# PaddlePaddle/MetaGym

Hardware: NVIDIA H100
Metric: env-steps/sec (quadrotor 6-DoF, 65k envs) (higher is better)
Workload: dtype f32

## Files before the change

metagym_b200/csrc/quad.cu:

```cuda
#include <math.h>
#include <stdlib.h>
#include <string.h>
#include <new>
#include <vector>

#include "mgb_common.cuh"
#include "quad_lanes.cuh"

namespace {

constexpr int kThreads = 64;
constexpr int kMaxObs = 19;

struct QuadConst {
    float h;
    float k1phi;
    float k1;
    float inv_phi;
    float hjm;
    float hk;
    float mm;
    float ct0, ct1, ct2;
    float vmin, vmax;
    float A[4], B[4];
// ... 691 lines not shown
    TargetRows<T> tr;
    int ct_now[N];
#pragma unroll
    for (int h = 0; h < N; ++h) {
        s.ct[h] += 1;
        ct_now[h] = s.ct[h];
    }
    const bool vel = c.task == MGB_TASK_VELOCITY_CONTROL;
    if (EARLY && vel) {
#pragma unroll
        for (int h = 0; h < N; ++h) prefetch_targets(c, a, task[h], ct_now[h], h, tr);
    }
    const T z_old = vadd(s.p[2], c.z_off);
    const T x_old = s.p[0], y_old = s.p[1];
    int fail[N];
    if (N == 1 && c.rk4_steps > 0) {
        QState s1;
        get_lane_state(s, 0, s1);
        float adj1[9], id1, pw1;
        fail[0] = integrate_rk4<SIMPLE>(c, s1, make_float4(lane(V[0], 0), lane(V[1], 0), lane(V[2], 0), lane(V[3], 0)),
                                        adj1, id1, pw1);
        set_lane_state(s, 0, s1);
#pragma unroll
        for (int k = 0; k < 9; ++k) set_lane(adj[k], 0, adj1[k]);
        set_lane(id, 0, id1);
        set_lane(power, 0, pw1);
    } else {
        const bool failed = integrate<SIMPLE, T>(c, s, V, adj, id, power, fail);
        if (N > 1 && failed) {
#pragma unroll 1
            for (int h = 0; h < N; ++h) {
                QState s1;
                load_state(a, e + h, s1);
                float adj1[9], id1, pw1;
                adjugate(s1.R, adj1, id1);
                const float V1[4] = {lane(V[0], h), lane(V[1], h), lane(V[2], h), lane(V[3], h)};
                int f1[1];
                integrate<SIMPLE, float>(c, s1, V1, adj1, id1, pw1, f1);
                s1.ct[0] = s.ct[h];
                s1.ep[0] = s.ep[h];
                set_lane_state(s, h, s1);
#pragma unroll
                for (int k = 0; k < 9; ++k) set_lane(adj[k], h, adj1[k]);
                set_lane(id, h, id1);
                set_lane(power, h, pw1);
                fail[h] = f1[0];
            }
        }
    }
    if (!EARLY && vel) {
#pragma unroll
        for (int h = 0; h < N; ++h) prefetch_targets(c, a, task[h], ct_now[h], h, tr);
    }
    const bool state_first = N == 1 && STATE_FIRST && vel;
    if (state_first) {
        QState s1;
        get_lane_state(s, 0, s1);
        if (s1.ct[0] == c.nt || fail[0]) s1.ct[0] = 0;
        store_state(a, e, s1);
    }
    T o[kMaxObs], reward;
    int done[N], trunc[N];
    bool wf[N];
    finish_step(c, a, e, s, adj, id, z_old, x_old, y_old, power, fail, tr, o, reward, done, wf, trunc);
    bool stored = false;
    if constexpr (N == 2) {
        if (nact == 2) {
            store_state2(a, e, s);
            *reinterpret_cast<float2 *>(a.rew + e) = reward.v;
            *reinterpret_cast<uchar2 *>(a.done + e) = make_uchar2((uint8_t)done[0], (uint8_t)done[1]);
            if (a.fail) *reinterpret_cast<int2 *>(a.fail + e) = make_int2(fail[0], fail[1]);
            if (a.truncated) *reinterpret_cast<uchar2 *>(a.truncated + e) = make_uchar2((uint8_t)trunc[0], (uint8_t)trunc[1]);
            stored = true;
        }
    }
    if (!stored) {
#pragma unroll
        for (int h = 0; h < N; ++h) {
            if (h < nact) {
                QState s1;
                get_lane_state(s, h, s1);
                if (!state_first || wf[h]) store_state(a, e + h, s1);
                a.rew[e + h] = lane(reward, h);
                a.done[e + h] = (uint8_t)done[h];
                if (a.fail) a.fail[e + h] = fail[h];
                if (a.truncated) a.truncated[e + h] = (uint8_t)trunc[h];
            }
        }
    }
#pragma unroll
    for (int h = 0; h < N; ++h) {
        if (h < nact) {
            float *tr_h = trow + h * D;
            if (wf[h]) {
                if (a.final_obs) {
                    float *fr_h = frow + h * D;
#pragma unroll
                    for (int k = 0; k < 16; ++k) fr_h[k] = lane(o[k], h);
                    if (D == 19) { fr_h[16] = lane(o[16], h); fr_h[17] = lane(o[17], h); fr_h[18] = lane(o[18], h); }
                    final_mask |= 1 << h;
                }
                observe_reset(c, a, task[h], s, h, o);
            }
#pragma unroll
            for (int k = 0; k < 16; ++k) tr_h[k] = lane(o[k], h);
            if (D == 19) { tr_h[16] = lane(o[16], h); tr_h[17] = lane(o[17], h); tr_h[18] = lane(o[18], h); }
        }
    }
}

__device__ __forceinline__ void publish_final(const QuadArgs &a, const float *ftile, int64_t e, int local_row, int lanes,
                                              int final_mask, int D)
{
    if (!a.final_obs) return;
    if (__syncthreads_or(final_mask)) {
        for (int h = 0; h < lanes; ++h) {
            if (final_mask & (1 << h)) {
                float *dst = a.final_obs + (e + h) * D;
                const float *frow = ftile + (local_row + h) * D;
                for (int k = 0; k < D; ++k) dst[k] = frow[k];
            }
        }
    }
}

template <bool SIMPLE>
__global__ void __launch_bounds__(kThreads) quad_step_kernel(const __grid_constant__ QuadConst c,
                                                             const __grid_constant__ QuadArgs a)
{
    __shared__ __align__(128) float tile[kThreads * kMaxObs];
    __shared__ __align__(128) float ftile[kThreads * kMaxObs];
    const int64_t e0 = (int64_t)blockIdx.x * kThreads;
    const int64_t e = e0 + threadIdx.x;
    const int rows = (int)((a.n - e0) < kThreads ? (a.n - e0) : kThreads);
    const int D = c.obs_dim;
    const bool active = e < a.n;
    int final_mask = 0;

    asm volatile("griddepcontrol.launch_dependents;");
    const int task[1] = {active ? env_task(c, a, e) : 0};
    asm volatile("griddepcontrol.wait;" ::: "memory");

    if (active) {
        QState s;
        load_state(a, e, s);
        const float4 act = __ldg(reinterpret_cast<const float4 *>(a.act) + e);
        const float V[4] = {act.x, act.y, act.z, act.w};
        step_body<SIMPLE, false, true, float>(c, a, e, 1, s, V, task, tile + threadIdx.x * D, ftile + threadIdx.x * D,
                                              final_mask);
    }
    publish_tile(a.obs, tile, e0, rows, D);
    publish_final(a, ftile, e, threadIdx.x, 1, final_mask, D);
    if (threadIdx.x == 0) mgb_bulk_wait_read<0>();
}

template <bool SIMPLE>
__global__ void __launch_bounds__(512, 1) quad_step_wide_kernel(const __grid_constant__ QuadConst c,
                                                                const __grid_constant__ QuadArgs a)
{
    extern __shared__ __align__(128) float wide_smem[];
    const int per = a.per_cta;
    float *tile = wide_smem, *ftile = wide_smem + (size_t)per * kMaxObs;
    const int64_t e0 = (int64_t)blockIdx.x * per;
    const int64_t e = e0 + threadIdx.x;
    int rows = (int)((a.n - e0) < per ? (a.n - e0) : per);
    if (rows < 0) rows = 0;
    const int D = c.obs_dim;
    const bool active = (int)threadIdx.x < rows;
    int final_mask = 0;
    asm volatile("griddepcontrol.launch_dependents;");
    const int task[1] = {active ? env_task(c, a, e) : 0};
    asm volatile("griddepcontrol.wait;" ::: "memory");
    if (active) {
        QState s;
        load_state(a, e, s);
        const float4 act = __ldg(reinterpret_cast<const float4 *>(a.act) + e);
        const float V[4] = {act.x, act.y, act.z, act.w};
        step_body<SIMPLE, false, false, float>(c, a, e, 1, s, V, task, tile + threadIdx.x * D, ftile + threadIdx.x * D,
                                               final_mask);
    }
    if (rows > 0) publish_tile(a.obs, tile, e0, rows, D);
    else __syncthreads();
    publish_final(a, ftile, e, threadIdx.x, 1, final_mask, D);
    if (threadIdx.x == 0) mgb_bulk_wait_read<0>();
}

template <bool SIMPLE>
__global__ void __launch_bounds__(256, 1) quad_step2_kernel(const __grid_constant__ QuadConst c,
                                                            const __grid_constant__ QuadArgs a)
{
    extern __shared__ __align__(128) float pair_smem[];
    const int per = a.per_cta;
    float *tile = pair_smem, *ftile = pair_smem + (size_t)per * kMaxObs;
    const int64_t e0 = (int64_t)blockIdx.x * per;
    int rows = (int)((a.n - e0) < per ? (a.n - e0) : per);
    if (rows < 0) rows = 0;
    const int le = 2 * (int)threadIdx.x;
    const int64_t e = e0 + le;
    const int D = c.obs_dim;
    const int nact = rows - le >= 2 ? 2 : (rows - le > 0 ? 1 : 0);
    int final_mask = 0;
    asm volatile("griddepcontrol.launch_dependents;");
    asm volatile("griddepcontrol.wait;" ::: "memory");
    if (nact > 0) {
        VState<f2> s;
        load_state2(a, e, s);
        const float4 a0 = __ldg(reinterpret_cast<const float4 *>(a.act) + e);
        const float4 a1 = nact == 2 ? __ldg(reinterpret_cast<const float4 *>(a.act) + e + 1) : make_float4(0.f, 0.f, 0.f, 0.f);
        const f2 V[4] = {pack2(a0.x, a1.x), pack2(a0.y, a1.y), pack2(a0.z, a1.z), pack2(a0.w, a1.w)};
        const int task[2] = {env_task(c, a, e), env_task(c, a, nact == 2 ? e + 1 : e)};
        step_body<SIMPLE, true, false, f2>(c, a, e, nact, s, V, task, tile + le * D, ftile + le * D, final_mask);
    }
    if (rows > 0) publish_tile(a.obs, tile, e0, rows, D);
    else __syncthreads();
    publish_final(a, ftile, e, le, 2, final_mask, D);
    if (threadIdx.x == 0) mgb_bulk_wait_read<0>();
}

constexpr int kStreamThreads = 128;

template <bool SIMPLE>
__global__ void __launch_bounds__(kStreamThreads, 4) quad_stream_kernel(const __grid_constant__ QuadConst c,
                                                                        const __grid_constant__ QuadArgs a)
{
    __shared__ __align__(128) float4 stage[2][7][kStreamThreads];
    __shared__ __align__(128) float tile[kStreamThreads * kMaxObs];
    __shared__ __align__(128) float ftile[kStreamThreads * kMaxObs];
    __shared__ __align__(8) uint64_t full[2];
    const int D = c.obs_dim;
    const int64_t n_tiles = (a.n + kStreamThreads - 1) / kStreamThreads;
    const int tid = threadIdx.x;

    asm volatile("griddepcontrol.launch_dependents;");
    asm volatile("griddepcontrol.wait;" ::: "memory");
    if (tid == 0) {
        mgb_mbar_init(&full[0], 1);
        mgb_mbar_init(&full[1], 1);
        mgb_fence_mbar_init();
    }
    __syncthreads();

    auto fetch = [&](int64_t t, int st) {
        const int64_t e0 = t * kStreamThreads;
        const uint32_t rows = (uint32_t)((a.n - e0) < kStreamThreads ? (a.n - e0) : kStreamThreads);
        static_assert(kStreamThreads == kTileEnvs, "one CTA iteration = one state tile");
        mgb_mbar_expect_tx(&full[st], 6u * kTileEnvs * 16u + rows * 16u);
        mgb_bulk_load(stage[st][0], a.planes + t * (6 * kTileEnvs), 6u * kTileEnvs * 16u, &full[st]);
        mgb_bulk_load(stage[st][6], reinterpret_cast<const float4 *>(a.act) + e0, rows * 16u, &full[st]);
    };

    int64_t t = blockIdx.x;
    if (tid == 0 && t < n_tiles) fetch(t, 0);
    uint32_t phase[2] = {0u, 0u};
    int st = 0;
    for (; t < n_tiles; t += gridDim.x, st ^= 1) {
        const int64_t t_next = t + gridDim.x;
        if (tid == 0 && t_next < n_tiles) fetch(t_next, st ^ 1);
        mgb_mbar_wait(&full[st], phase[st]);
        phase[st] ^= 1u;
        const int64_t e0 = t * kStreamThreads, e = e0 + tid;
        const int rows = (int)((a.n - e0) < kStreamThreads ? (a.n - e0) : kStreamThreads);
        int final_mask = 0;
        if (tid == 0) mgb_bulk_wait_read<0>();
        __syncthreads();
        if (tid < rows) {
            QState s;
            float4 q[kPlanes];
#pragma unroll
            for (int k = 0; k < kPlanes; ++k) q[k] = stage[st][k][tid];
            unpack_state(q, s);
            const float4 act = stage[st][6][tid];
            const float V[4] = {act.x, act.y, act.z, act.w};
            const int task[1] = {env_task(c, a, e)};
            step_body<SIMPLE, true, false, float>(c, a, e, 1, s, V, task, tile + tid * D, ftile + tid * D, final_mask);
        }
        publish_tile(a.obs, tile, e0, rows, D);
        publish_final(a, ftile, e, tid, 1, final_mask, D);
        __syncthreads();
    }
    if (tid == 0) mgb_bulk_wait_read<0>();
}

template <bool SIMPLE, int XM, bool FIN>
__global__ void __launch_bounds__(kThreads, 8) quad_rollout_kernel(const __grid_constant__ QuadConst c,
                                                                const __grid_constant__ QuadArgs a)
{
    __shared__ __align__(128) float tiles[2][kThreads * kMaxObs];
    const int64_t e0 = (int64_t)blockIdx.x * kThreads;
    const int64_t e = e0 + threadIdx.x;
    const int rows = (int)((a.n - e0) < kThreads ? (a.n - e0) : kThreads);
    const int D = c.obs_dim;
    const bool active = e < a.n;
    QState s;
    float adj[9], id = 1.f;
    if (active) {
        load_state(a, e, s);
        adjugate(s.R, adj, id);
    }
    const uint2 akey = make_uint2((uint32_t)a.act_seed, (uint32_t)(a.act_seed >> 32));
    const int64_t genv = a.env_base + e;
    const int task = active ? env_task(c, a, e) : 0;
    float4 act_next = make_float4(0.f, 0.f, 0.f, 0.f);
    if (active && a.act) act_next = __ldg(reinterpret_cast<const float4 *>(a.act) + e);
    for (int t = 0; t < a.T; ++t) {
        float *tile = tiles[t & 1];
        if (threadIdx.x == 0) mgb_bulk_wait_read<1>();
// ... 50 lines not shown
                if (XM == 1) mgb_mirror_store(a.mir, a.rew + (int64_t)t * a.n + e, reward);
            }
            done_byte = (uint32_t)done[0];
            if (a.done && XM != 2) {
                a.done[(int64_t)t * a.n + e] = (uint8_t)done[0];
                if (XM == 1) mgb_mirror_store(a.mir, a.done + (int64_t)t * a.n + e, (uint8_t)done[0]);
            }
            if (a.obs) {
                float *orow = tile + threadIdx.x * D;
#pragma unroll
                for (int k = 0; k < 16; ++k) orow[k] = o[k];
                if (D == 19) { orow[16] = o[16]; orow[17] = o[17]; orow[18] = o[18]; }
            }
        }
        if (XM == 2) {
            if (a.done) mgb_mc_st_bytes(mgb_shift(a.done + (int64_t)t * a.n + e, a.mir.delta[0]), done_byte, active);
            if (a.obs) {
                __syncthreads();
                mgb_mc_copy_tile(mgb_shift(a.obs + ((int64_t)t * a.n + e0) * D, a.mir.delta[0]), tile,
                                 (uint32_t)rows * (uint32_t)D * 4u);
            }
        } else if (a.obs) {
            if (XM == 1) publish_tile_mirrored(a.mir, a.obs + (int64_t)t * a.n * D, tile, e0, rows, D);
            else publish_tile(a.obs + (int64_t)t * a.n * D, tile, e0, rows, D);
        }
    }
    if (active) store_state(a, e, s);
    if (threadIdx.x == 0) mgb_bulk_wait_read<0>();
}

__global__ void __launch_bounds__(kThreads) quad_reset_kernel(const __grid_constant__ QuadConst c,
                                                              const __grid_constant__ QuadArgs a,
                                                              const uint8_t *__restrict__ mask,
                                                              const double *__restrict__ noise)
{
    const int64_t e = (int64_t)blockIdx.x * kThreads + threadIdx.x;
    if (e >= a.n) return;
    QState s;
    load_state(a, e, s);
    if (!mask || mask[e]) {
        double u[12];
        if (noise) {
#pragma unroll
            for (int k = 0; k < 12; ++k) u[k] = noise[e * 12 + k];
        } else {
            s.ep[0] += 1;
            philox_reset_draws(a.seed, a.env_base + e, s.ep[0], u);
        }
        reset_env(c, s, 0, u);
        store_state(a, e, s);
    }
    if (a.obs) {
        float adj[9], id, o[kMaxObs], bv[3], Ri[9];
        adjugate(s.R, adj, id);
        observe(c, s, adj, id, o, bv, Ri);
        if (c.task == MGB_TASK_VELOCITY_CONTROL) {
            const float4 q = target_row(a, env_task(c, a, e), s.ct[0] < c.nt - 1 ? s.ct[0] : c.nt - 1);
            o[16] = q.x; o[17] = q.y; o[18] = q.z;
        }
        float *dst = a.obs + e * c.obs_dim;
#pragma unroll
        for (int k = 0; k < 16; ++k) dst[k] = o[k];
        if (c.obs_dim == 19) { dst[16] = o[16]; dst[17] = o[17]; dst[18] = o[18]; }
    }
}

__global__ void quad_state_kernel(QuadArgs a, float *state, int32_t *ct, int load)
{
    const int64_t e = (int64_t)blockIdx.x * blockDim.x + threadIdx.x;
    if (e >= a.n) return;
    QState s;
    load_state(a, e, s);
    float *row = state + e * 22;
    if (load) {
        for (int k = 0; k < 3; ++k) { s.p[k] = row[k]; s.v[k] = row[3 + k]; s.om[k] = row[6 + k]; }
        for (int k = 0; k < 4; ++k) s.w[k] = row[9 + k];
        for (int k = 0; k < 9; ++k) s.R[k] = row[13 + k];
        if (ct) s.ct[0] = ct[e];
        store_state(a, e, s);
    } else {
        for (int k = 0; k < 3; ++k) { row[k] = s.p[k]; row[3 + k] = s.v[k]; row[6 + k] = s.om[k]; }
        for (int k = 0; k < 4; ++k) row[9 + k] = s.w[k];
        for (int k = 0; k < 9; ++k) row[13 + k] = s.R[k];
        if (ct) ct[e] = s.ct[0];
    }
}

__global__ void quad_init_kernel(QuadArgs a)
{
    const int64_t e = (int64_t)blockIdx.x * blockDim.x + threadIdx.x;
    if (e >= a.n_pad) return;
    QState s;
    for (int k = 0; k < 3; ++k) s.p[k] = s.v[k] = s.om[k] = 0.f;
    for (int k = 0; k < 4; ++k) s.w[k] = 0.f;
    for (int k = 0; k < 9; ++k) s.R[k] = (k % 4 == 0) ? 1.f : 0.f;
    s.ct[0] = 0;
    s.ep[0] = 0;
    store_state(a, e, s);
}

template <bool SIMPLE>
__global__ void quad_targets_kernel(const __grid_constant__ QuadConst c, const float *__restrict__ act, int n_tasks,
                                    float *__restrict__ tbl)
{
    const int k = blockIdx.x * blockDim.x + threadIdx.x;
    if (k >= n_tasks) return;
    QState s;
    for (int q = 0; q < 3; ++q) s.p[q] = s.v[q] = s.om[q] = 0.f;
    for (int q = 0; q < 4; ++q) s.w[q] = 0.f;
    for (int q = 0; q < 9; ++q) s.R[q] = (q % 4 == 0) ? 1.f : 0.f;
    s.ct[0] = 0; s.ep[0] = 0;
    float adj[9], id, power;
    adjugate(s.R, adj, id);
    for (int t = 0; t < c.nt; ++t) {
        const float4 a4 = reinterpret_cast<const float4 *>(act)[(int64_t)k * c.nt + t];
        const int fail = integrate1<SIMPLE>(c, s, a4, adj, id, power);
        float *dst = tbl + ((int64_t)k * c.nt + t) * 3;
        dst[0] = s.v[0]; dst[1] = s.v[1]; dst[2] = s.v[2];
        if (fail) {
            for (int r = t + 1; r < c.nt; ++r) {
                float *d2 = tbl + ((int64_t)k * c.nt + r) * 3;
                d2[0] = d2[1] = d2[2] = __int_as_float(0x7fc00000);
            }
            return;
        }
    }
}

__global__ void quad_targets_layout_kernel(const float *__restrict__ src, int nt, int n_tasks, float4 *__restrict__ dst)
{
    const int64_t i = (int64_t)blockIdx.x * blockDim.x + threadIdx.x;
    if (i >= (int64_t)nt * n_tasks) return;
    const int64_t t = i / n_tasks, k = i % n_tasks;
    const float *s = src + (k * nt + t) * 3;
    dst[i] = make_float4(s[0], s[1], s[2], 0.f);
}

}

struct mgb_quad {
    int device = 0;
    int64_t n = 0, n_pad = 0, env_base = 0;
    mgb_quad_cfg cfg;
    QuadConst c;
    float4 *planes = nullptr;
    int32_t *sat = nullptr;
    int map_rows = 0, map_cols = 0, x_off = 0, y_off = 0;
    float4 *targets = nullptr;
    int32_t *env2task = nullptr;
    int n_tasks = 0;
    int auto_reset = 0;
    int num_sms = 132;
    int wide_kernel = -1;
    int packed = 0;
    int stream_kernel = 1;
    int pdl = 1;
    int zerocopy = 1;
    uint64_t seed = 0;
    uint32_t t_base = 0;
    int64_t launches = 0;
    MgbMirrors mir = {};
    MgbMirrorWindow mir_win;
    float *h_act = nullptr, *h_obs = nullptr, *h_rew = nullptr, *h_final = nullptr;
    uint8_t *h_done = nullptr, *h_trunc = nullptr;
    int32_t *h_fail = nullptr;
    float *d_act = nullptr, *d_obs = nullptr, *d_rew = nullptr, *d_final = nullptr;
    uint8_t *d_done = nullptr, *d_trunc = nullptr;
    int32_t *d_fail = nullptr;
};

static QuadArgs base_args(const mgb_quad *h)
{
    QuadArgs a;
    memset(&a, 0, sizeof(a));
    a.planes = h->planes;
    a.n_pad = h->n_pad;
    a.n = h->n;
    a.env_base = h->env_base;
    a.targets = h->targets;
    a.n_tasks = h->n_tasks;
    a.sat = h->sat; a.map_rows = h->map_rows; a.map_cols = h->map_cols; a.x_off = h->x_off; a.y_off = h->y_off;
    a.env2task = h->env2task;
    a.seed = h->seed;
    a.auto_reset = h->auto_reset;
    return a;
}

static int derive_constants(const mgb_quad_cfg *g, QuadConst *c)
{
    memset(c, 0, sizeof(*c));
    c->h = (float)g->precision;
    c->k1 = (float)(g->phi / g->ra);
    c->k1phi = (float)(g->phi / g->ra * g->phi);
    c->inv_phi = (float)(1.0 / g->phi);
    c->hjm = (float)(g->precision / g->jm);
    c->hk = (float)(g->precision / g->jm * (g->phi / g->ra * g->phi));
    c->mm = (float)g->mm;
    c->ct0 = (float)g->ct[0]; c->ct1 = (float)g->ct[1]; c->ct2 = (float)g->ct[2];
    c->vmin = (float)g->min_voltage; c->vmax = (float)g->max_voltage;
    bool simple = (g->ct[2] == 0.0);
    for (int i = 0; i < 4; ++i) {
        c->px[i] = g->propeller[3 * i]; c->py[i] = g->propeller[3 * i + 1]; c->pz[i] = g->propeller[3 * i + 2];
        c->A[i] = (float)((double)c->py[i] * (double)g->propeller_norm[i]);
        c->B[i] = (float)((double)c->px[i] * (double)g->propeller_norm[i]);
        if (c->pz[i] != 0.f) simple = false;
    }
    for (int k = 0; k < 3; ++k) {
        c->Df[k] = g->drag_f[k]; c->Dm[k] = g->drag_m[k]; c->cg[k] = g->gravity_center[k];
        if (c->cg[k] != 0.f) simple = false;
        c->init_v[k] = g->init_velocity[k]; c->init_w[k] = g->init_angular_velocity[k];
    }
    for (int k = 0; k < 9; ++k) {
        c->hI[k] = (float)(g->precision * (double)g->inv_inertia[k]);
        if (k % 4 != 0 && g->inv_inertia[k] != 0.f) simple = false;
    }
    c->gm = (float)((double)(float)-9.8 * g->quality);
    c->c_hm = (float)(g->precision / g->quality);
    c->c_h2m = (float)(0.5 * g->precision * g->precision / g->quality);
    c->fail_r2 = (float)(g->fail_range * g->fail_range);
    c->fail_v2 = (float)(g->fail_velocity * g->fail_velocity);
    c->fail_w2 = (float)(g->fail_w * g->fail_w);
    c->dt = (float)g->dt; c->healthy = (float)g->healthy_reward; c->z_off = (float)g->z_offset;
    c->noise_v = (float)g->init_velocity_noise; c->noise_w = (float)g->init_angular_velocity_noise;
    c->nt = g->nt; c->task = g->task;
    c->substeps = (int)(g->dt / g->precision);
    c->rk4_steps = g->integrator == MGB_INTEGRATOR_RK4 ? (g->rk4_steps > 0 ? g->rk4_steps : 1) : 0;
    c->rk4_h = c->rk4_steps ? (float)(g->dt / c->rk4_steps) : 0.f;
    c->inv_jm = (float)(1.0 / g->jm);
    c->inv_m = (float)(1.0 / g->quality);
    for (int k = 0; k < 9; ++k) c->Iinv[k] = g->inv_inertia[k];
    c->obs_dim = g->task == MGB_TASK_VELOCITY_CONTROL ? 19 : 16;
    c->simple = simple ? 1 : 0;
    return 0;
}

extern "C" int mgb_quad_create(mgb_quad **out, int64_t n_envs, const mgb_quad_cfg *cfg, int device,
                               int64_t env_index_base)
{
    MGB_REQUIRE(out && cfg, "null argument");
    MGB_REQUIRE(n_envs > 0, "n_envs must be positive");
    MGB_REQUIRE(cfg->task >= 0 && cfg->task <= 2, "invalid task");
    MGB_REQUIRE(cfg->nt > 0, "nt must be positive");
    MGB_REQUIRE(!(cfg->precision < 1e-8 || cfg->precision > cfg->dt), "Inproper parameter of precision");
    int ndev = 0;
    MGB_CUDA(cudaGetDeviceCount(&ndev));
    MGB_REQUIRE(device >= 0 && device < ndev, "device index out of range");
    MgbDeviceGuard guard(device);
    mgb_quad *h = new (std::nothrow) mgb_quad();
    MGB_REQUIRE(h, "out of host memory");
    h->device = device;
    h->n = n_envs;
    h->n_pad = (n_envs + 127) / 128 * 128;
    h->env_base = env_index_base;
    h->cfg = *cfg;
    derive_constants(cfg, &h->c);
    if (const char *ev = getenv("MGB_PDL")) h->pdl = atoi(ev) != 0;
    {
        cudaDeviceProp prop;
        if (cudaGetDeviceProperties(&prop, device) == cudaSuccess) h->num_sms = prop.multiProcessorCount;
    }
    if (const char *ev = getenv("MGB_HOST_ZEROCOPY")) h->zerocopy = atoi(ev);
    if (const char *ev = getenv("MGB_STREAM_KERNEL")) h->stream_kernel = atoi(ev) != 0;
    if (const char *ev = getenv("MGB_PACKED")) h->packed = atoi(ev) != 0;
    if (const char *ev = getenv("MGB_WIDE_KERNEL")) h->wide_kernel = atoi(ev) != 0;
    {
        const int max_smem = 512 * kMaxObs * 4 * 2;
        cudaFuncSetAttribute(quad_step_wide_kernel<true>, cudaFuncAttributeMaxDynamicSharedMemorySize, max_smem);
        cudaFuncSetAttribute(quad_step_wide_kernel<false>, cudaFuncAttributeMaxDynamicSharedMemorySize, max_smem);
        cudaFuncSetAttribute(quad_step2_kernel<true>, cudaFuncAttributeMaxDynamicSharedMemorySize, max_smem);
        cudaFuncSetAttribute(quad_step2_kernel<false>, cudaFuncAttributeMaxDynamicSharedMemorySize, max_smem);
        if (cudaGetLastError() != cudaSuccess) {
            mgb_set_error("cudaFuncSetAttribute(quad_step_wide_kernel, %d bytes of shared memory) failed", max_smem);
            delete h;
            return MGB_ERR_CUDA;
        }
    }
    cudaError_t e = cudaMalloc(&h->planes, sizeof(float4) * 6 * h->n_pad);
    if (e != cudaSuccess) {
        mgb_set_error("cudaMalloc(state planes, %lld envs) -> %s", (long long)n_envs, cudaGetErrorString(e));
        delete h;
        return MGB_ERR_CUDA;
    }
    QuadArgs a = base_args(h);
    quad_init_kernel<<<(unsigned)((h->n_pad + 255) / 256), 256>>>(a);
    e = cudaDeviceSynchronize();
    if (e != cudaSuccess) {
        mgb_set_error("state init -> %s", cudaGetErrorString(e));
        cudaFree(h->planes);
        delete h;
        return MGB_ERR_CUDA;
    }
    h->launches += 1;
    *out = h;
    return MGB_OK;
}

extern "C" void mgb_quad_destroy(mgb_quad *h)
{
    if (!h) return;
    MgbDeviceGuard guard(h->device);
    cudaDeviceSynchronize();
    cudaFree(h->planes);
    cudaFree(h->sat);
    cudaFree(h->targets);
    cudaFree(h->env2task);
    cudaFree(h->d_act); cudaFree(h->d_obs); cudaFree(h->d_rew); cudaFree(h->d_done);
    cudaFree(h->d_fail); cudaFree(h->d_final); cudaFree(h->d_trunc);
    cudaFreeHost(h->h_act); cudaFreeHost(h->h_obs); cudaFreeHost(h->h_rew); cudaFreeHost(h->h_done);
    cudaFreeHost(h->h_fail); cudaFreeHost(h->h_final); cudaFreeHost(h->h_trunc);
    delete h;
}

extern "C" int mgb_quad_obs_dim(const mgb_quad *h) { return h ? h->c.obs_dim : MGB_ERR_ARG; }
extern "C" int64_t mgb_quad_num_envs(const mgb_quad *h) { return h ? h->n : MGB_ERR_ARG; }
extern "C" int64_t mgb_quad_launch_count(const mgb_quad *h) { return h ? h->launches : MGB_ERR_ARG; }

extern "C" int mgb_quad_set_options(mgb_quad *h, int auto_reset, uint64_t seed)
{
    MGB_REQUIRE(h, "null handle");
    h->auto_reset = auto_reset ? 1 : 0;
    h->seed = seed;
    return MGB_OK;
}

extern "C" int mgb_quad_set_map(mgb_quad *h, const int32_t *map_host, int32_t rows, int32_t cols)
{
    MGB_REQUIRE(h, "null handle");
    MgbDeviceGuard guard(h->device);
    MGB_CUDA(cudaDeviceSynchronize());
    cudaFree(h->sat);
    h->sat = nullptr;
    h->map_rows = h->map_cols = h->x_off = h->y_off = 0;
    if (!map_host) return MGB_OK;
    MGB_REQUIRE(h->c.task != MGB_TASK_VELOCITY_CONTROL, "velocity_control has no map (env.py:101-104)");
    MGB_REQUIRE(rows > 0 && cols > 0 && rows <= 8192 && cols <= 8192, "map size out of range");
    int starts = 0, sr = 0, sc = 0;
    for (int r = 0; r < rows; ++r)
        for (int q = 0; q < cols; ++q)
            if (map_host[(size_t)r * cols + q] == -1) { ++starts; sr = r; sc = q; }
    MGB_REQUIRE(starts == 1, "the map must mark exactly one start cell with -1 (env.py:108-109)");
    std::vector<int32_t> sat((size_t)(rows + 1) * (cols + 1), 0);
    for (int r = 0; r < rows; ++r)
        for (int q = 0; q < cols; ++q) {
            const int v = (r == sr && q == sc) ? 0 : map_host[(size_t)r * cols + q];
            sat[(size_t)(r + 1) * (cols + 1) + q + 1] = (v != 0 ? 1 : 0) + sat[(size_t)r * (cols + 1) + q + 1] +
                                                        sat[(size_t)(r + 1) * (cols + 1) + q] - sat[(size_t)r * (cols + 1) + q];
        }
    MGB_CUDA(cudaMalloc(&h->sat, sat.size() * sizeof(int32_t)));
    MGB_CUDA(cudaMemcpy(h->sat, sat.data(), sat.size() * sizeof(int32_t), cudaMemcpyHostToDevice));
    h->map_rows = rows; h->map_cols = cols; h->x_off = sc; h->y_off = sr;
    return MGB_OK;
}

extern "C" int mgb_quad_set_targets(mgb_quad *h, const float *tbl_dev, int32_t n_tasks, const int32_t *env2task_dev)
{
    MGB_REQUIRE(h && tbl_dev && env2task_dev, "null argument");
    MGB_REQUIRE(n_tasks > 0, "n_tasks must be positive");
    MgbDeviceGuard guard(h->device);
    MGB_CUDA(cudaDeviceSynchronize());
    cudaFree(h->targets); h->targets = nullptr;
    cudaFree(h->env2task); h->env2task = nullptr;
    h->n_tasks = 0;
    const int64_t rows = (int64_t)h->c.nt * n_tasks;
    MGB_CUDA(cudaMalloc(&h->targets, sizeof(float4) * (size_t)rows));
    MGB_CUDA(cudaMalloc(&h->env2task, sizeof(int32_t) * h->n));
    quad_targets_layout_kernel<<<(unsigned)((rows + 255) / 256), 256>>>(tbl_dev, h->c.nt, n_tasks, h->targets);
    MGB_CUDA(cudaGetLastError());
    MGB_CUDA(cudaMemcpy(h->env2task, env2task_dev, sizeof(int32_t) * h->n, cudaMemcpyDeviceToDevice));
    MGB_CUDA(cudaDeviceSynchronize());
    h->n_tasks = n_tasks;
    return MGB_OK;
}

static int check_ready(const mgb_quad *h)
{
    if (h->c.task == MGB_TASK_VELOCITY_CONTROL && !h->targets) {
        mgb_set_error("velocity_control: call mgb_quad_set_targets before reset/step");
        return MGB_ERR_STATE;
    }
    return MGB_OK;
}

extern "C" int mgb_quad_make_targets(mgb_quad *h, const float *act_dev, int32_t n_tasks, float *tbl_dev, void *stream)
{
    MgbRange nvtx_range("mgb_quad_make_targets");
    MGB_REQUIRE(h && act_dev && tbl_dev, "null argument");
    MGB_REQUIRE(n_tasks > 0, "n_tasks must be positive");
    MgbDeviceGuard guard(h->device);
    cudaStream_t st = (cudaStream_t)stream;
    const int threads = 32, blocks = (n_tasks + threads - 1) / threads;
    if (h->c.simple) quad_targets_kernel<true><<<blocks, threads, 0, st>>>(h->c, act_dev, n_tasks, tbl_dev);
    else quad_targets_kernel<false><<<blocks, threads, 0, st>>>(h->c, act_dev, n_tasks, tbl_dev);
    MGB_CUDA(cudaGetLastError());
    h->launches += 1;
    return MGB_OK;
}

extern "C" int mgb_quad_reset(mgb_quad *h, const uint8_t *mask_dev, const double *noise_dev, float *obs_dev,
                              void *stream)
{
    MgbRange nvtx_range("mgb_quad_reset");
    MGB_REQUIRE(h, "null handle");
    int rc = check_ready(h);
    if (rc) return rc;
    MgbDeviceGuard guard(h->device);
    QuadArgs a = base_args(h);
    a.obs = obs_dev;
    quad_reset_kernel<<<(unsigned)((h->n + kThreads - 1) / kThreads), kThreads, 0, (cudaStream_t)stream>>>(
        h->c, a, mask_dev, noise_dev);
    MGB_CUDA(cudaGetLastError());
    h->launches += 1;
    return MGB_OK;
}

enum StepKernel { STEP_TILE = 0, STEP_WIDE = 1, STEP_STREAM = 2, STEP_PACKED = 3 };

static StepKernel choose_step_kernel(const mgb_quad *h, const QuadArgs &a)
{
    const unsigned blocks = (unsigned)((a.n + kThreads - 1) / kThreads);
    const bool act16 = (reinterpret_cast<uintptr_t>(a.act) & 15u) == 0;
    if (h->stream_kernel && (int64_t)blocks > (int64_t)h->num_sms * 32 && act16) return STEP_STREAM;
    if (h->packed && h->c.rk4_steps == 0 && a.n >= 2) {
        const bool aligned = act16 && (reinterpret_cast<uintptr_t>(a.rew) & 7u) == 0 &&
                             (reinterpret_cast<uintptr_t>(a.done) & 1u) == 0 && (reinterpret_cast<uintptr_t>(a.fail) & 7u) == 0 &&
                             (reinterpret_cast<uintptr_t>(a.truncated) & 1u) == 0;
        if (aligned) return STEP_PACKED;
    }
    const bool single_wave = a.n <= (int64_t)h->num_sms * 512 && a.n >= (int64_t)h->num_sms * 64;
    const int64_t wide_max = (int64_t)h->num_sms * (h->wide_kernel > 0 ? 512 : 384);
    if (h->wide_kernel != 0 && single_wave && a.n <= wide_max) return STEP_WIDE;
    return STEP_TILE;
}

static int launch_step(mgb_quad *h, const QuadArgs &a, cudaStream_t st)
{
    const unsigned blocks = (unsigned)((a.n + kThreads - 1) / kThreads);
    cudaLaunchConfig_t cfg;
    memset(&cfg, 0, sizeof(cfg));
    cfg.gridDim = dim3(blocks);
    cfg.blockDim = dim3(kThreads);
    cfg.stream = st;
    cudaLaunchAttribute attr[1];
    attr[0].id = cudaLaunchAttributeProgrammaticStreamSerialization;
    attr[0].val.programmaticStreamSerializationAllowed = h->pdl ? 1 : 0;
    cfg.attrs = attr;
    cfg.numAttrs = 1;
    const StepKernel which = choose_step_kernel(h, a);
    if (which == STEP_STREAM) {
        cfg.gridDim = dim3((unsigned)(h->num_sms * 4));
        cfg.blockDim = dim3(kStreamThreads);
        if (h->c.simple) MGB_CUDA(cudaLaunchKernelEx(&cfg, quad_stream_kernel<true>, h->c, a));
        else MGB_CUDA(cudaLaunchKernelEx(&cfg, quad_stream_kernel<false>, h->c, a));
    } else if (which == STEP_WIDE || which == STEP_PACKED) {
        const int lanes = which == STEP_PACKED ? 2 : 1;
        int per;
        if (a.n <= (int64_t)h->num_sms * 512 && a.n >= (int64_t)h->num_sms * 64) per = (int)((a.n + h->num_sms - 1) / h->num_sms);
        else per = a.n < (int64_t)h->num_sms * 64 ? 64 : 256;
        per = (per + 3) / 4 * 4;
        QuadArgs aw = a;
        aw.per_cta = per;
        cfg.gridDim = dim3((unsigned)((a.n + per - 1) / per));
        cfg.blockDim = dim3((unsigned)((per / lanes + 31) / 32 * 32));
        cfg.dynamicSmemBytes = (size_t)per * kMaxObs * 4 * 2;
        if (which == STEP_PACKED) {
            if (h->c.simple) MGB_CUDA(cudaLaunchKernelEx(&cfg, quad_step2_kernel<true>, h->c, aw));
            else MGB_CUDA(cudaLaunchKernelEx(&cfg, quad_step2_kernel<false>, h->c, aw));
        } else {
            if (h->c.simple) MGB_CUDA(cudaLaunchKernelEx(&cfg, quad_step_wide_kernel<true>, h->c, aw));
            else MGB_CUDA(cudaLaunchKernelEx(&cfg, quad_step_wide_kernel<false>, h->c, aw));
        }
    } else {
        if (h->c.simple) MGB_CUDA(cudaLaunchKernelEx(&cfg, quad_step_kernel<true>, h->c, a));
        else MGB_CUDA(cudaLaunchKernelEx(&cfg, quad_step_kernel<false>, h->c, a));
    }
    MGB_CUDA(cudaGetLastError());
    h->launches += 1;
    return MGB_OK;
}

extern "C" const char *mgb_quad_step_kernel(const mgb_quad *h)
{
    if (!h) return "";
    QuadArgs a = base_args(h);
    switch (choose_step_kernel(h, a)) {
    case STEP_STREAM: return h->c.simple ? "quad_stream_kernel<true>" : "quad_stream_kernel<false>";
    case STEP_PACKED: return h->c.simple ? "quad_step2_kernel<true>" : "quad_step2_kernel<false>";
    case STEP_WIDE: return h->c.simple ? "quad_step_wide_kernel<true>" : "quad_step_wide_kernel<false>";
    default: return h->c.simple ? "quad_step_kernel<true>" : "quad_step_kernel<false>";
    }
}

static int step_dev(mgb_quad *h, const float *act_dev, float *obs_dev, float *rew_dev, uint8_t *done_dev,
                    int32_t *fail_dev, float *final_obs_dev, uint8_t *truncated_dev, void *stream)
{
    MGB_REQUIRE(h && act_dev && obs_dev && rew_dev && done_dev, "null argument");
    MGB_REQUIRE((reinterpret_cast<uintptr_t>(act_dev) & 15u) == 0, "act_dev must be 16-byte aligned");
    int rc = check_ready(h);
    if (rc) return rc;
    MgbDeviceGuard guard(h->device);
    QuadArgs a = base_args(h);
    a.act = act_dev; a.obs = obs_dev; a.rew = rew_dev; a.done = done_dev; a.fail = fail_dev;
    a.final_obs = final_obs_dev;
    a.truncated = truncated_dev;
    return launch_step(h, a, (cudaStream_t)stream);
}

extern "C" int mgb_quad_step(mgb_quad *h, const float *act_dev, float *obs_dev, float *rew_dev, uint8_t *done_dev,
                             int32_t *fail_dev, float *final_obs_dev, void *stream)
{
    MgbRange nvtx_range("mgb_quad_step");
    return step_dev(h, act_dev, obs_dev, rew_dev, done_dev, fail_dev, final_obs_dev, nullptr, stream);
}

extern "C" int mgb_quad_step_ex(mgb_quad *h, const float *act_dev, float *obs_dev, float *rew_dev, uint8_t *done_dev,
                                int32_t *fail_dev, float *final_obs_dev, uint8_t *truncated_dev, void *stream)
{
    MgbRange nvtx_range("mgb_quad_step_ex");
    return step_dev(h, act_dev, obs_dev, rew_dev, done_dev, fail_dev, final_obs_dev, truncated_dev, stream);
}

static int rollout(mgb_quad *h, int32_t T, const float *act_dev, uint64_t act_seed, float *act_out_dev, float *obs_dev,
                   float *rew_dev, uint8_t *done_dev, float *final_obs_dev, uint8_t *truncated_dev, void *stream)
{
    MGB_REQUIRE(h, "null handle");
    MGB_REQUIRE(T > 0, "T must be positive");
    MGB_REQUIRE((reinterpret_cast<uintptr_t>(act_dev) & 15u) == 0, "act_dev must be 16-byte aligned");
    const bool fin = final_obs_dev || truncated_dev;
    MGB_REQUIRE(!final_obs_dev || h->auto_reset, "final_obs needs auto_reset on (without it obs already is the terminal observation)");
    MGB_REQUIRE(!fin || h->mir.count == 0,
                "final_obs / truncated are not delivered through output mirrors or multicast (set_mirrors([]) first)");
    int rc = check_ready(h);
    if (rc) return rc;
    MgbDeviceGuard guard(h->device);
    QuadArgs a = base_args(h);
    a.act = act_dev; a.obs = obs_dev; a.rew = rew_dev; a.done = done_dev;
    a.T = T; a.act_seed = act_seed; a.t_base = h->t_base; a.act_out = act_out_dev;
    a.final_obs = final_obs_dev; a.truncated = truncated_dev;
    const unsigned blocks = (unsigned)((a.n + kThreads - 1) / kThreads);
    a.mir = h->mir;
    if (h->mir.count != 0)
        MGB_REQUIRE(h->mir_win.holds(obs_dev, (uint64_t)T * h->n * h->c.obs_dim * 4) &&
                        h->mir_win.holds(rew_dev, (uint64_t)T * h->n * 4) && h->mir_win.holds(done_dev, (uint64_t)T * h->n) &&
                        h->mir_win.holds(act_out_dev, (uint64_t)T * h->n * 16),
                    "mirrors are on but an output lies outside the mirrored arena (set_mirrors([]) first)");
    if (h->mir.count == MGB_MIRROR_MULTICAST) {
        MGB_REQUIRE(h->n % 4 == 0, "multicast outputs need num_envs % 4 == 0");
        MGB_REQUIRE((((uintptr_t)done_dev | (uintptr_t)rew_dev | (uintptr_t)obs_dev) & 3) == 0 && ((uintptr_t)act_out_dev & 15) == 0,
                    "multicast outputs must be 4-byte (actions: 16-byte) aligned");
        if (h->c.simple) quad_rollout_kernel<true, 2, false><<<blocks, kThreads, 0, (cudaStream_t)stream>>>(h->c, a);
        else quad_rollout_kernel<false, 2, false><<<blocks, kThreads, 0, (cudaStream_t)stream>>>(h->c, a);
    } else if (h->mir.count > 0) {
        if (h->c.simple) quad_rollout_kernel<true, 1, false><<<blocks, kThreads, 0, (cudaStream_t)stream>>>(h->c, a);
        else quad_rollout_kernel<false, 1, false><<<blocks, kThreads, 0, (cudaStream_t)stream>>>(h->c, a);
    } else if (fin) {
        if (h->c.simple) quad_rollout_kernel<true, 0, true><<<blocks, kThreads, 0, (cudaStream_t)stream>>>(h->c, a);
        else quad_rollout_kernel<false, 0, true><<<blocks, kThreads, 0, (cudaStream_t)stream>>>(h->c, a);
    } else {
        if (h->c.simple) quad_rollout_kernel<true, 0, false><<<blocks, kThreads, 0, (cudaStream_t)stream>>>(h->c, a);
        else quad_rollout_kernel<false, 0, false><<<blocks, kThreads, 0, (cudaStream_t)stream>>>(h->c, a);
    }
    MGB_CUDA(cudaGetLastError());
    h->t_base += (uint32_t)T;
    h->launches += 1;
    return MGB_OK;
}

extern "C" int mgb_quad_rollout(mgb_quad *h, int32_t T, const float *act_dev, uint64_t act_seed, float *act_out_dev,
                                float *obs_dev, float *rew_dev, uint8_t *done_dev, void *stream)
{
    MgbRange nvtx_range("mgb_quad_rollout");
    return rollout(h, T, act_dev, act_seed, act_out_dev, obs_dev, rew_dev, done_dev, nullptr, nullptr, stream);
}

extern "C" int mgb_quad_rollout_ex(mgb_quad *h, int32_t T, const float *act_dev, uint64_t act_seed, float *act_out_dev,
                                   float *obs_dev, float *rew_dev, uint8_t *done_dev, float *final_obs_dev,
                                   uint8_t *truncated_dev, void *stream)
{
    MgbRange nvtx_range("mgb_quad_rollout_ex");
    return rollout(h, T, act_dev, act_seed, act_out_dev, obs_dev, rew_dev, done_dev, final_obs_dev, truncated_dev,
                   stream);
}

extern "C" int mgb_quad_set_mirrors(mgb_quad *h, int count, const int64_t *byte_delta)
{
    MGB_REQUIRE(h, "null handle");
    MGB_REQUIRE(count >= 0 && count <= MGB_MAX_MIRRORS && (count == 0 || byte_delta), "count out of range");
    MgbMirrors m = {};
    for (int i = 0; i < count; ++i) {
        MGB_REQUIRE((byte_delta[i] & 15) == 0, "mirror deltas must be multiples of 16 bytes");
        m.delta[i] = byte_delta[i];
    }
    m.count = count;
    h->mir = m;
    return MGB_OK;
}

extern "C" int mgb_quad_set_mirror_window(mgb_quad *h, const void *base, uint64_t bytes)
{
    MGB_REQUIRE(h, "null handle");
    h->mir_win.base = reinterpret_cast<uintptr_t>(base);
    h->mir_win.bytes = bytes;
    return MGB_OK;
}

extern "C" int mgb_quad_set_multicast(mgb_quad *h, int64_t byte_delta)
{
    MGB_REQUIRE(h, "null handle");
    MGB_REQUIRE((byte_delta & 15) == 0, "multicast delta must be a multiple of 16 bytes");
    MgbMirrors m = {};
    if (byte_delta != 0) { m.count = MGB_MIRROR_MULTICAST; m.delta[0] = byte_delta; }
    h->mir = m;
    return MGB_OK;
}

static int ensure_host_staging(mgb_quad *h)
{
    if (h->d_act) return MGB_OK;
    const size_t n = (size_t)h->n, D = (size_t)h->c.obs_dim;
    MGB_CUDA(cudaMalloc(&h->d_act, n * 16));
    MGB_CUDA(cudaMalloc(&h->d_obs, n * D * 4));
    MGB_CUDA(cudaMalloc(&h->d_rew, n * 4));
    MGB_CUDA(cudaMalloc(&h->d_done, n));
    MGB_CUDA(cudaMalloc(&h->d_fail, n * 4));
    MGB_CUDA(cudaMalloc(&h->d_final, n * D * 4));
    MGB_CUDA(cudaMalloc(&h->d_trunc, n));
    MGB_CUDA(cudaMallocHost(&h->h_trunc, n));
    MGB_CUDA(cudaMemset(h->d_fail, 0, n * 4));
    MGB_CUDA(cudaMemset(h->d_final, 0, n * D * 4));
    MGB_CUDA(cudaMallocHost(&h->h_act, n * 16));
    MGB_CUDA(cudaMallocHost(&h->h_obs, n * D * 4));
    MGB_CUDA(cudaMallocHost(&h->h_rew, n * 4));
    MGB_CUDA(cudaMallocHost(&h->h_done, n));
    MGB_CUDA(cudaMallocHost(&h->h_fail, n * 4));
    MGB_CUDA(cudaMallocHost(&h->h_final, n * D * 4));
    return MGB_OK;
}

static void *pinned_device_alias(const void *p)
{
    cudaPointerAttributes at;
// ... 97 lines not shown
```

Baseline: 8.516 billion.

## Add two-cohort step kernel with staggered loads and per-cohort bulk stores

Adds a 256-thread step kernel that splits each CTA into two 128-env cohorts. The second cohort waits on a named barrier until the first cohort has issued its state and action loads, so the two cohorts' memory traffic is staggered. Each cohort publishes its observation tile through its own named barrier and bulk async store, so the halves do not wait on each other. It is selected by default for single-wave sizes of at least 65536 envs, which replaces the 64-thread tile kernel at this size; the gate serialises part of the load phase and may cost occupancy.

Result: faster. 8.886 billion, median of 6 (+4.3%).

```diff
diff --git a/metagym_b200/csrc/quad.cu b/metagym_b200/csrc/quad.cu
--- a/metagym_b200/csrc/quad.cu
+++ b/metagym_b200/csrc/quad.cu
@@ -867,6 +867,88 @@
     publish_tile(a.obs, tile, e0, rows, D);
     publish_final(a, ftile, e, threadIdx.x, 1, final_mask, D);
     if (threadIdx.x == 0) mgb_bulk_wait_read<0>();
+}
+
+constexpr int kGateBar = 1, kCohortBar = 2;
+
+template <int ID, int COUNT> __device__ __forceinline__ void named_bar_sync()
+{
+    asm volatile("bar.sync %0, %1;" ::"n"(ID), "n"(COUNT) : "memory");
+}
+
+template <int BAR, int COUNT>
+__device__ __forceinline__ void publish_cohort_tile(float *gobs, const float *tile, int64_t e0, int rows, int D, int lt)
+{
+    const uint32_t bytes = (uint32_t)rows * (uint32_t)D * 4u;
+    float *dst = gobs + e0 * D;
+    if ((bytes & 15u) == 0 && ((reinterpret_cast<uintptr_t>(dst) & 15u) == 0)) {
+        mgb_fence_proxy_async();
+        named_bar_sync<BAR, COUNT>();
+        if (lt == 0) {
+            mgb_bulk_store(dst, tile, bytes);
+            mgb_bulk_commit();
+        }
+    } else {
+        named_bar_sync<BAR, COUNT>();
+        for (int i = lt; i < rows * D; i += COUNT) dst[i] = tile[i];
+    }
+}
+
+constexpr int kCohortEnvs = 128;
+
+template <bool SIMPLE>
+__global__ void __launch_bounds__(2 * kCohortEnvs, 2) quad_step_kernel_cohorts(const __grid_constant__ QuadConst c,
+                                                                               const __grid_constant__ QuadArgs a)
+{
+    constexpr int kCta = 2 * kCohortEnvs;
+    __shared__ __align__(128) float tile[kCta * kMaxObs];
+    __shared__ __align__(128) float ftile[kCta * kMaxObs];
+    const int cohort = (int)threadIdx.x / kCohortEnvs;
+    const int lt = (int)threadIdx.x % kCohortEnvs;
+    const int64_t c0 = (int64_t)blockIdx.x * kCta + cohort * kCohortEnvs;
+    const int64_t e = c0 + lt;
+    const int rows = (int)((a.n - c0) < kCohortEnvs ? ((a.n - c0) > 0 ? (a.n - c0) : 0) : kCohortEnvs);
+    const int D = c.obs_dim;
+    const bool active = e < a.n;
+    float *ctile = tile + cohort * kCohortEnvs * D, *cftile = ftile + cohort * kCohortEnvs * D;
+    int final_mask = 0;
+
+    asm volatile("griddepcontrol.launch_dependents;");
+    const int task[1] = {active ? env_task(c, a, e) : 0};
+    asm volatile("griddepcontrol.wait;" ::: "memory");
+
+    if (cohort == 1) named_bar_sync<kGateBar, kCta>();
+    float4 q[kPlanes], act;
+    if (active) {
+        const float4 *b = tile_base(a, e);
+#pragma unroll
+        for (int k = 0; k < kPlanes; ++k) q[k] = b[k * kTileEnvs];
+        act = __ldg(reinterpret_cast<const float4 *>(a.act) + e);
+    } else {
+#pragma unroll
+        for (int k = 0; k < kPlanes; ++k) q[k] = make_float4(0.f, 0.f, 0.f, 0.f);
+        act = make_float4(0.f, 0.f, 0.f, 0.f);
+    }
+    if (cohort == 0) {
+        asm volatile("bar.arrive %0, %1;" ::"n"(kGateBar), "n"(kCta), "f"(q[0].x), "f"(q[1].x), "f"(q[2].x), "f"(q[3].x),
+                     "f"(q[4].x), "f"(q[5].x), "f"(act.x)
+                     : "memory");
+    }
+    if (active) {
+        QState s;
+        unpack_state(q, s);
+        const float V[4] = {act.x, act.y, act.z, act.w};
+        step_body<SIMPLE, false, true, float>(c, a, e, 1, s, V, task, ctile + lt * D, cftile + lt * D, final_mask);
+    }
+    if (rows > 0) {
+        if (cohort == 0) publish_cohort_tile<kCohortBar, kCohortEnvs>(a.obs, ctile, c0, rows, D, lt);
+        else publish_cohort_tile<kCohortBar + 1, kCohortEnvs>(a.obs, ctile, c0, rows, D, lt);
+    }
+    if (final_mask) {
+        const float *frow = cftile + lt * D;
+        for (int k = 0; k < D; ++k) a.final_obs[e * D + k] = frow[k];
+    }
+    if (lt == 0) mgb_bulk_wait_read<0>();
 }
 
 template <bool SIMPLE>
@@ -1223,6 +1305,7 @@
     int auto_reset = 0;
     int num_sms = 132;
     int wide_kernel = -1;
+    int cohort_kernel = -1;
     int packed = 0;
     int stream_kernel = 1;
     int pdl = 1;
@@ -1334,6 +1417,7 @@
     if (const char *ev = getenv("MGB_STREAM_KERNEL")) h->stream_kernel = atoi(ev) != 0;
     if (const char *ev = getenv("MGB_PACKED")) h->packed = atoi(ev) != 0;
     if (const char *ev = getenv("MGB_WIDE_KERNEL")) h->wide_kernel = atoi(ev) != 0;
+    if (const char *ev = getenv("MGB_COHORT_KERNEL")) h->cohort_kernel = atoi(ev) != 0;
     {
         const int max_smem = 512 * kMaxObs * 4 * 2;
         cudaFuncSetAttribute(quad_step_wide_kernel<true>, cudaFuncAttributeMaxDynamicSharedMemorySize, max_smem);
@@ -1484,7 +1568,7 @@
     return MGB_OK;
 }
 
-enum StepKernel { STEP_TILE = 0, STEP_WIDE = 1, STEP_STREAM = 2, STEP_PACKED = 3 };
+enum StepKernel { STEP_TILE = 0, STEP_WIDE = 1, STEP_STREAM = 2, STEP_PACKED = 3, STEP_COHORT = 4 };
 
 static StepKernel choose_step_kernel(const mgb_quad *h, const QuadArgs &a)
 {
@@ -1500,6 +1584,8 @@
     const bool single_wave = a.n <= (int64_t)h->num_sms * 512 && a.n >= (int64_t)h->num_sms * 64;
     const int64_t wide_max = (int64_t)h->num_sms * (h->wide_kernel > 0 ? 512 : 384);
     if (h->wide_kernel != 0 && single_wave && a.n <= wide_max) return STEP_WIDE;
+    if (h->cohort_kernel > 0 || (h->cohort_kernel < 0 && h->wide_kernel != 0 && single_wave && a.n >= 65536))
+        return STEP_COHORT;
     return STEP_TILE;
 }
 
@@ -1540,6 +1626,11 @@
             if (h->c.simple) MGB_CUDA(cudaLaunchKernelEx(&cfg, quad_step_wide_kernel<true>, h->c, aw));
             else MGB_CUDA(cudaLaunchKernelEx(&cfg, quad_step_wide_kernel<false>, h->c, aw));
         }
+    } else if (which == STEP_COHORT) {
+        cfg.gridDim = dim3((unsigned)((a.n + 2 * kCohortEnvs - 1) / (2 * kCohortEnvs)));
+        cfg.blockDim = dim3(2 * kCohortEnvs);
+        if (h->c.simple) MGB_CUDA(cudaLaunchKernelEx(&cfg, quad_step_kernel_cohorts<true>, h->c, a));
+        else MGB_CUDA(cudaLaunchKernelEx(&cfg, quad_step_kernel_cohorts<false>, h->c, a));
     } else {
         if (h->c.simple) MGB_CUDA(cudaLaunchKernelEx(&cfg, quad_step_kernel<true>, h->c, a));
         else MGB_CUDA(cudaLaunchKernelEx(&cfg, quad_step_kernel<false>, h->c, a));
@@ -1557,6 +1648,7 @@
     case STEP_STREAM: return h->c.simple ? "quad_stream_kernel<true>" : "quad_stream_kernel<false>";
     case STEP_PACKED: return h->c.simple ? "quad_step2_kernel<true>" : "quad_step2_kernel<false>";
     case STEP_WIDE: return h->c.simple ? "quad_step_wide_kernel<true>" : "quad_step_wide_kernel<false>";
+    case STEP_COHORT: return h->c.simple ? "quad_step_kernel_cohorts<true>" : "quad_step_kernel_cohorts<false>";
     default: return h->c.simple ? "quad_step_kernel<true>" : "quad_step_kernel<false>";
     }
 }
```
